# xyfJASON/ctrlora

Hardware: AMD Instinct MI355X
Metric: 512x512 LoRA-finetune images/sec (higher is better)
Workload: dtype bf16; 1 GPU; ctrlora_finetune_sd15_rank128.yaml, canny-style latent hint, 512x512 (latent 64x64), per-GPU batch 8, bf16 storage / fp32 accumulate, synthetic latents + random-init weights, LoRA+zero-conv+norm trainables, fused AdamW; global_batch=8, parallelism=dp1, lora_rank=128, launch=hipGraph replay, gemm_launch_table_entries=215

## Files before the change

ctrlora_amd/csrc/gemm.hip:

```cpp
#include <type_traits>
#include "gemm.h"
#include <algorithm>
#include <cstring>
#include <map>
#include <vector>
#include <utility>
#include "mma.h"
#include "gemm_epi.h"

namespace cl {

static void* g_ws = nullptr;
static long g_ws_bytes = 0;
struct StreamWs { hipStream_t st; void* p; long bytes; };
static StreamWs g_sws[4] = {};
static thread_local hipStream_t t_stream = nullptr;
void gemm_set_workspace(void* p, long bytes) { g_ws = p; g_ws_bytes = bytes; }
int gemm_set_stream_workspace(hipStream_t st, void* p, long bytes) {
  for (auto& e : g_sws) if (e.st == st || e.p == nullptr) { e.st = st; e.p = p; e.bytes = bytes; return CL_OK; }
  return CL_EINVAL;
}
static void ws_for(hipStream_t st, void** p, long* bytes) {
  for (auto& e : g_sws) if (e.p && e.st == st) { *p = e.p; *bytes = e.bytes; return; }
  *p = g_ws; *bytes = g_ws_bytes;
}
void gemm_get_workspace(void** p, long* bytes) { ws_for(t_stream, p, bytes); }
void gemm_get_workspace_for(hipStream_t st, void** p, long* bytes) { ws_for(st, p, bytes); }

int g_gemm_tag_on = 0;
static thread_local int t_tag = 0;
struct TagEntry { long v[12]; };
static std::vector<TagEntry> g_tags;
int gemm_cur_tag() { return t_tag; }
void gemm_tag_note(long real_wgs, int wg_size) {
  if (t_tag > 0 && t_tag <= (int)g_tags.size()) { g_tags[t_tag - 1].v[9] = real_wgs; g_tags[t_tag - 1].v[10] = wg_size; }
}
int gemm_tag_count() { return (int)g_tags.size(); }
void gemm_tag_clear() { g_tags.clear(); t_tag = 0; }
int gemm_tag_get(int i, long* out) {
  if (i < 0 || i >= (int)g_tags.size()) return CL_EINVAL;
  for (int k = 0; k < 12; ++k) out[k] = g_tags[i].v[k];
// ... 72 lines not shown
          }
        }
        __syncthreads();
        continue;
      }
    }
    __builtin_amdgcn_wave_barrier();
    asm volatile("s_waitcnt lgkmcnt(0)" ::: "memory");
#pragma unroll
    for (int it = 0; it < ITERS; ++it) {
      const int rr = it * RPI + lane / LPR;
      const int cg = (lane % LPR) * 8;
      const int grow = row0 + ps * 32 + rr;
      const int gcol = col0 + cg;
      if (lane < RPI * LPR && rr < FPP * 16 && grow < p.M && gcol < p.N) {
        float v[8];
        const float4 s0 = *reinterpret_cast<const float4*>(&stg[rr * EST + cg]);
        const float4 s1 = *reinterpret_cast<const float4*>(&stg[rr * EST + cg + 4]);
        v[0] = s0.x; v[1] = s0.y; v[2] = s0.z; v[3] = s0.w;
        v[4] = s1.x; v[5] = s1.y; v[6] = s1.z; v[7] = s1.w;
        if (slab) {
          store8(slab + ((long)zsplit * p.M + grow) * p.N + gcol, v);
        } else if (p.act != 77) {
          epilogue8<T>(e, v, grow, gcol);
        }
      }
    }
    __builtin_amdgcn_wave_barrier();
  }
}

template <typename T, int BM, int BN, int WGM, int WGN, int KSUB, int R>
__global__ __launch_bounds__(WGM * WGN * 64, 2) void gemm_kernel(GemmParams p, int tiles_m, int tiles_n,
                                                              float* __restrict__ slab) {
  constexpr int NW = WGM * WGN;
  constexpr int KPB = 64 / (int)sizeof(T);
  constexpr int WM = BM / WGM, WN = BN / WGN, FM = WM / 16, FN = WN / 16;
  constexpr int AG = BM / 16, BG = BN / 16;
  constexpr int AJ = AG / NW, BJ = (BG + NW - 1) / NW;
  constexpr int G = AJ + BJ;
  constexpr int D = R - KSUB;
  constexpr int SLOT = (AG + BG) * 1024;
  constexpr int EST = WN + 4;
  constexpr int EROWS = (FM >= 2) ? 32 : 16;
  constexpr int EPI_BYTES = NW * EROWS * EST * 4;
  constexpr int SMEM = (R * SLOT > EPI_BYTES) ? R * SLOT : EPI_BYTES;
  static_assert(AG % NW == 0 && WM % 16 == 0 && WN % 16 == 0 && WN % 8 == 0, "tile shape");
  static_assert(D >= KSUB && D >= 1, "ring too shallow");
  static_assert(FM == 1 || FM % 2 == 0, "FM");
  extern __shared__ __attribute__((aligned(16))) char smem[];

  const int tid = threadIdx.x, lane = tid & 63;
  const int wave = __builtin_amdgcn_readfirstlane(tid >> 6);
  const int wm = wave / WGN, wn = wave % WGN;

  const int nt = tiles_m * tiles_n;
  if ((int)blockIdx.x >= nt * max(p.splitk, 1)) return;
  int pid = blockIdx.x;
  const int zsplit = pid / nt;
  pid -= zsplit * nt;
  {
    const int q = nt >> 3, r = nt & 7, xcd = pid & 7, idx = pid >> 3;
    pid = (xcd < r ? xcd * (q + 1) : r * (q + 1) + (xcd - r) * q) + idx;
  }
  const int m0 = (pid / tiles_n) * BM, n0 = (pid % tiles_n) * BN;

  const int taps = (p.mode == GEMM_LINEAR) ? 1 : 9;
  const int cpt = p.K1 / KPB;
  const int ks1 = taps * cpt;
  const int ks2 = p.K2 / KPB;
  int kbeg = 0, kend = ks1 + ks2;
  if (p.splitk > 1) {
    const int per = (kend + p.splitk - 1) / p.splitk;
    kbeg = zsplit * per;
    kend = min(kend, kbeg + per);
  }

  const int lrow = lane >> 2;
  const int lchk = (lane & 3) * 16;
  const char* a1[AJ]; const char* a2[AJ];
  int ab[AJ], ay[AJ], ax[AJ];
#pragma unroll
  for (int j = 0; j < AJ; ++j) {
    int r = m0 + (j * NW + wave) * 16 + lrow;
    r = min(r, p.M - 1);
    a2[j] = p.A2 ? (const char*)p.A2 + ((long)r * p.lda2 + (p.a2_group_n ? (long)(n0 / p.a2_group_n) * p.K2 : 0)) * sizeof(T) + lchk
                 : nullptr;
    if (p.mode == GEMM_LINEAR) {
      a1[j] = (const char*)p.A1 + ((long)r * p.lda1 + (p.a1_group_n ? (long)(n0 / p.a1_group_n) * p.K1 : 0)) * sizeof(T) + lchk;
      ab[j] = ay[j] = ax[j] = 0;
    } else {
      const int ox = r % p.Wout; const int t = r / p.Wout;
      ax[j] = ox; ay[j] = t % p.Hout; ab[j] = t / p.Hout;
      a1[j] = (const char*)p.A1 + lchk;
    }
  }
  const char* w1[BJ]; const char* w2[BJ];
  int bgrp[BJ];
#pragma unroll
  for (int j = 0; j < BJ; ++j) {
    bgrp[j] = min(j * NW + wave, BG - 1);
    int n = n0 + bgrp[j] * 16 + lrow;
    n = min(n, p.N - 1);
    w1[j] = (const char*)p.W1 + ((long)n * p.ldw1) * sizeof(T) + lchk;
    w2[j] = p.W2 ? (const char*)p.W2 + ((long)n * p.ldw2) * sizeof(T) + lchk : nullptr;
  }
  const char* zpage = (const char*)p.zero_page + lchk;

  auto issue = [&](int kt, int slot) {
    char* As = smem + slot * SLOT;
    char* Bs = As + AG * 1024;
    const bool seg2 = kt >= ks1;
    const long koff = (long)(seg2 ? kt - ks1 : kt) * 64;
    if (seg2 || p.mode == GEMM_LINEAR) {
#pragma unroll
      for (int j = 0; j < AJ; ++j) glds16((seg2 ? a2[j] : a1[j]) + koff, As + (j * NW + wave) * 1024);
    } else {
      const int tap = kt / cpt, cc = kt - tap * cpt;
      const int ky = tap / 3, kx = tap - ky * 3;
      const int sy = (p.mode == GEMM_CONV_S2 || p.mode == GEMM_CONV_S2A) ? 2 : 1;
      const int po = (p.mode == GEMM_CONV_S2A) ? 0 : 1;
      const bool virt = (p.mode == GEMM_CONV_UP2) | (p.mode == GEMM_CONV_T2);
#pragma unroll
      for (int j = 0; j < AJ; ++j) {
        const int vy = ay[j] * sy + ky - po, vx = ax[j] * sy + kx - po;
        bool ok; int iy, ix;
        if (virt) {
          ok = ((unsigned)vy < (unsigned)(2 * p.Hin)) & ((unsigned)vx < (unsigned)(2 * p.Win));
          if (p.mode == GEMM_CONV_T2) ok = ok & !((vy | vx) & 1);
          iy = vy >> 1; ix = vx >> 1;
        } else {
          ok = ((unsigned)vy < (unsigned)p.Hin) & ((unsigned)vx < (unsigned)p.Win);
          iy = vy; ix = vx;
        }
        const long pix = ((long)ab[j] * p.Hin + iy) * p.Win + ix;
        const char* src = ok ? a1[j] + (pix * p.lda1 + (long)cc * KPB) * sizeof(T) : zpage;
        glds16(src, As + (j * NW + wave) * 1024);
      }
    }
#pragma unroll
    for (int j = 0; j < BJ; ++j) glds16((seg2 ? w2[j] : w1[j]) + koff, Bs + bgrp[j] * 1024);
  };

  f32x4_t acc[FM][FN];
#pragma unroll
  for (int i = 0; i < FM; ++i)
#pragma unroll
    for (int j = 0; j < FN; ++j) acc[i][j] = f32x4_t{0.f, 0.f, 0.f, 0.f};

  const int frag_off = ((lane & 15) * 4 + (lane >> 4)) * 16;
  const uint32_t lds_base = (uint32_t)(uintptr_t)smem;
  const uint32_t a_frag = lds_base + (wm * FM) * 1024 + frag_off;
// ... 50 lines not shown
      const bool two = it + 1 < total;
      read_frags(it % R, af0, bf0);
      wait_frags(af0, bf0);
      if (two) read_frags((it + 1) % R, af1, bf1);
      __builtin_amdgcn_sched_barrier(0);
      mma_all(af0, bf0);
      if (two) {
        wait_frags(af1, bf1);
        mma_all(af1, bf1);
      }
    }
  }
  __syncthreads();

  store_tile<T, FM, FN, (WGN == 2 && FN == 5)>(p, acc, reinterpret_cast<float*>(smem) + wave * (EROWS * EST),
                                               m0 + wm * WM, n0 + wn * WN, lane, slab, zsplit, wn,
                                               reinterpret_cast<float*>(smem) + (wave ^ 1) * (EROWS * EST));
}

enum { FL_LINEAR = 0, FL_CONV_S1 = 1, FL_CONV_ANY = 2 };

#ifdef FL_TIMING
__device__ unsigned long long* g_fl_timing = nullptr;
#define FL_STAMP(i) do { if (g_fl_timing && threadIdx.x == 0) { g_fl_timing[(long)vpid * 8 + (i)] = __builtin_amdgcn_s_memtime(); \
    if ((i) == 0) { g_fl_timing[(long)vpid * 8 + 5] = __builtin_amdgcn_s_getreg((31 << 11) | 4);     \
                    g_fl_timing[(long)vpid * 8 + 6] = __builtin_amdgcn_s_getreg((31 << 11) | 20); } } } while (0)
void fl_timing_set(unsigned long long* buf) { (void)hipMemcpyToSymbol(HIP_SYMBOL(g_fl_timing), &buf, sizeof(buf)); }
#else
#define FL_STAMP(i) do { } while (0)
#endif

template <typename T, int BM, int BN, int WGM, int WGN, int MODE, int R, int PRIO>
__device__ __forceinline__ void fl_tile(const GemmParams& p, int tiles_m, int tiles_n, float* __restrict__ slab,
                                        int vpid, char* smem) {
  constexpr int NW = WGM * WGN;
  static_assert(R == 2 || R == 3, "ring depth");
  constexpr int KPS = 128 / (int)sizeof(T);
  constexpr int WM = BM / WGM, WN = BN / WGN, FM = WM / 16, FN = WN / 16;
  constexpr int AI = BM / 8, BI = BN / 8;
  constexpr int AJ = AI / NW, BJ = (BI + NW - 1) / NW;
  constexpr int G = AJ + BJ;
  constexpr int SLOT = (AI + BI) * 1024;
  constexpr int EST = WN + 4;
  constexpr int EROWS = (FM >= 2) ? 32 : 16;
  static_assert(AI % NW == 0 && WM % 16 == 0 && WN % 16 == 0, "tile shape");
  static_assert(NW * EROWS * EST * 4 <= R * SLOT, "epilogue staging must fit in the ring");
  FL_STAMP(0);

  const int tid = threadIdx.x, lane = tid & 63;
  const int wave = __builtin_amdgcn_readfirstlane(tid >> 6);
  const int wm = wave / WGN, wn = wave % WGN;

  const int nt = tiles_m * tiles_n;
  int pid = vpid;
  const int zsplit = pid / nt;
  pid -= zsplit * nt;
  {
    const int q = nt >> 3, r = nt & 7, xcd = pid & 7, idx = pid >> 3;
    pid = (xcd < r ? xcd * (q + 1) : r * (q + 1) + (xcd - r) * q) + idx;
  }
  const int m0 = (pid / tiles_n) * BM, n0 = (pid % tiles_n) * BN;

  const int cpt = p.K1 / KPS;
  int ph_mq = 0, ph = 0, ph_ntx = 3, ph_dy0 = 0, ph_dx0 = 0, ntaps = (MODE == FL_CONV_ANY && p.mode == GEMM_CONV_S2K4) ? 16 : 9;
  long ph_woff = 0;
  if constexpr (MODE == FL_CONV_ANY) {
    if (gemm_phase_mode(p.mode)) {
      ph_mq = p.B * p.Hin * p.Win;
      ph = m0 / ph_mq;
      const int a = ph >> 1, b = ph & 1;
      if (p.mode == GEMM_CONV_UP2P) { ph_ntx = 2; ntaps = 4; ph_dy0 = a - 1; ph_dx0 = b - 1; ph_woff = (long)ph * 4 * p.N * p.K1; }
      else { ph_ntx = 1 + b; ntaps = (1 + a) * (1 + b); ph_woff = (long)p.N * p.K1 * (ph == 0 ? 0 : ph == 1 ? 1 : ph == 2 ? 3 : 5); }
    }
  }
  const long ldw1 = ph_mq ? (long)ntaps * p.K1 : p.ldw1;
  const int ks1 = (MODE == FL_LINEAR ? 1 : ntaps) * cpt;
  const int ks2 = (MODE == FL_LINEAR) ? p.K2 / KPS : 0;
  int kbeg = 0, kend = ks1 + ks2;
  if (p.splitk > 1) {
    const int per = (kend + p.splitk - 1) / p.splitk;
    kbeg = zsplit * per;
    kend = min(kend, kbeg + per);
  }
  const int total = kend - kbeg;

  const int lrow = lane >> 3, lslot = lane & 7;
  const char* pa[AJ];
  const char* a2[AJ];
  uint32_t vmask[AJ];
  int ab[AJ], ay[AJ], ax[AJ];
#pragma unroll
  for (int j = 0; j < AJ; ++j) {
    const int inst = j * NW + wave;
    const int chunk = (lslot ^ (((inst & 1) << 2) | (lrow >> 1))) * 16;
    int r = m0 + inst * 8 + lrow;
    r = min(r, p.M - 1);
    a2[j] = nullptr; vmask[j] = 0; ab[j] = ay[j] = ax[j] = 0;
    if constexpr (MODE == FL_LINEAR) {
      const bool in2 = kbeg >= ks1;
      a2[j] = p.A2 ? (const char*)p.A2 + ((long)r * p.lda2 + (p.a2_group_n ? (long)(n0 / p.a2_group_n) * p.K2 : 0)) * sizeof(T) + chunk
                   : nullptr;
      pa[j] = in2 ? a2[j] + (long)(kbeg - ks1) * 128
                  : (const char*)p.A1 + ((long)r * p.lda1 + (p.a1_group_n ? (long)(n0 / p.a1_group_n) * p.K1 : 0)) * sizeof(T) +
                        chunk + (long)kbeg * 128;
    } else {
      const int rq = ph_mq ? r - ph * ph_mq : r;
      const int gw = ph_mq ? p.Win : p.Wout, gh = ph_mq ? p.Hin : p.Hout;
      const int ox = rq % gw; const int t = rq / gw;
      const int oy = t % gh, ob = t / gh;
      if constexpr (MODE == FL_CONV_S1) {
        pa[j] = (const char*)p.A1 + ((((long)ob * p.Hin + oy) * p.Win + ox) * p.lda1) * sizeof(T) + chunk;
        uint32_t m = 0;
#pragma unroll
        for (int tp = 0; tp < 9; ++tp) {
          const int vy = oy + tp / 3 - 1, vx = ox + tp % 3 - 1;
          if (((unsigned)vy < (unsigned)p.Hin) & ((unsigned)vx < (unsigned)p.Win)) m |= 1u << tp;
        }
        vmask[j] = m;
      } else {
        pa[j] = (const char*)p.A1 + chunk;
        ax[j] = ox; ay[j] = oy; ab[j] = ob;
      }
    }
  }
  const char* pw[BJ]; const char* w2[BJ];
  int binst[BJ];
#pragma unroll
  for (int j = 0; j < BJ; ++j) {
    binst[j] = min(j * NW + wave, BI - 1);
    const int chunk = (lslot ^ (((binst[j] & 1) << 2) | (lrow >> 1))) * 16;
    int n = n0 + binst[j] * 8 + lrow;
    n = min(n, p.N - 1);
    w2[j] = (MODE == FL_LINEAR && p.W2) ? (const char*)p.W2 + ((long)n * p.ldw2) * sizeof(T) + chunk : nullptr;
    pw[j] = (MODE == FL_LINEAR && kbeg >= ks1)
                ? w2[j] + (long)(kbeg - ks1) * 128
                : (const char*)p.W1 + (ph_woff + (long)n * ldw1) * sizeof(T) + chunk + (long)kbeg * 128;
  }
  const char* zpage = (const char*)p.zero_page + lslot * 16;

  int kt_next = kbeg;
  int tap = (MODE == FL_LINEAR) ? 0 : kbeg / cpt;
  int cc = (MODE == FL_LINEAR) ? 0 : kbeg - tap * cpt;
  const long pixb = (long)p.lda1 * sizeof(T);
  long tapoff = 0;
  const char* cur[AJ];
#pragma unroll
  for (int j = 0; j < AJ; ++j) cur[j] = nullptr;
  if constexpr (MODE == FL_CONV_S1) {
    tapoff = ((long)(tap / 3 - 1) * p.Win + (tap % 3 - 1)) * pixb;
#pragma unroll
    for (int j = 0; j < AJ; ++j)
      cur[j] = ((vmask[j] >> tap) & 1u) ? pa[j] + tapoff + (long)cc * 128 : zpage + (long)cc * 128;
  }

  auto issue_a = [&](int slot) {
    char* As = smem + slot * SLOT;
    if constexpr (MODE == FL_LINEAR) {
      if (ks2 && kt_next == ks1) {
#pragma unroll
        for (int j = 0; j < AJ; ++j) pa[j] = a2[j];
      }
#pragma unroll
      for (int j = 0; j < AJ; ++j) { glds16(pa[j], As + (j * NW + wave) * 1024); pa[j] += 128; }
    } else if constexpr (MODE == FL_CONV_S1) {
      if (cc == 0) {
#pragma unroll
        for (int j = 0; j < AJ; ++j) cur[j] = ((vmask[j] >> tap) & 1u) ? pa[j] + tapoff : zpage;
      }
#pragma unroll
      for (int j = 0; j < AJ; ++j) { glds16(cur[j], As + (j * NW + wave) * 1024); cur[j] += 128; }
    } else {
      const bool k4 = p.mode == GEMM_CONV_S2K4;
      const int ky = k4 ? tap >> 2 : tap / 3, kx = k4 ? tap & 3 : tap - ky * 3;
      const int sy = (p.mode == GEMM_CONV_S2 || p.mode == GEMM_CONV_S2A || k4) ? 2 : 1;
      const int po = (p.mode == GEMM_CONV_S2A) ? 0 : 1;
      const bool virt = (p.mode == GEMM_CONV_UP2) | (p.mode == GEMM_CONV_T2);
      const int pty = ph_ntx == 2 ? tap >> 1 : tap, ptx = ph_ntx == 2 ? tap & 1 : 0;
#pragma unroll
      for (int j = 0; j < AJ; ++j) {
        const int vy = ph_mq ? ay[j] + ph_dy0 + pty : ay[j] * sy + ky - po;
        const int vx = ph_mq ? ax[j] + ph_dx0 + ptx : ax[j] * sy + kx - po;
        bool ok; int iy, ix;
        if (virt) {
          ok = ((unsigned)vy < (unsigned)(2 * p.Hin)) & ((unsigned)vx < (unsigned)(2 * p.Win));
          if (p.mode == GEMM_CONV_T2) ok = ok & !((vy | vx) & 1);
          iy = vy >> 1; ix = vx >> 1;
        } else {
          ok = ((unsigned)vy < (unsigned)p.Hin) & ((unsigned)vx < (unsigned)p.Win);
          iy = vy; ix = vx;
        }
        const long pix = ((long)ab[j] * p.Hin + iy) * p.Win + ix;
        const char* src = ok ? pa[j] + pix * pixb + (long)cc * 128 : zpage;
        glds16(src, As + (j * NW + wave) * 1024);
      }
    }
  };
  auto issue_b = [&](int slot) {
    char* Bs = smem + slot * SLOT + AI * 1024;
    if constexpr (MODE == FL_LINEAR) {
      if (ks2 && kt_next == ks1) {
#pragma unroll
        for (int j = 0; j < BJ; ++j) pw[j] = w2[j];
      }
    } else if constexpr (MODE == FL_CONV_S1) {
      const bool wrap = cc + 1 == cpt;
      cc = wrap ? 0 : cc + 1;
      tap += wrap ? 1 : 0;
      const int ky = (tap * 11) >> 5;
      tapoff = ((long)(ky - 1) * p.Win + (tap - 3 * ky - 1)) * pixb;
    } else {
      if (++cc == cpt) { cc = 0; ++tap; }
    }
#pragma unroll
    for (int j = 0; j < BJ; ++j) { glds16(pw[j], Bs + binst[j] * 1024); pw[j] += 128; }
    ++kt_next;
  };
  auto issue_next = [&](int slot) { issue_a(slot); issue_b(slot); };
  FL_STAMP(1);

  f32x4_t acc[FM][FN];
#pragma unroll
  for (int i = 0; i < FM; ++i)
#pragma unroll
    for (int j = 0; j < FN; ++j) acc[i][j] = f32x4_t{0.f, 0.f, 0.f, 0.f};

  const int lr = lane & 15, g = lane >> 4;
  const uint32_t lds_base = (uint32_t)(uintptr_t)smem;
  const uint32_t frag0 = lr * 128 + ((g ^ (lr >> 1)) * 16);
  const uint32_t a_base = lds_base + (wm * FM) * 2048;
  const uint32_t b_base = lds_base + AI * 1024 + (wn * FN) * 2048;

  auto read_frags = [&](int slot, int half, u32x4_t (&af)[FM], u32x4_t (&bfr)[FN]) {
    const uint32_t off = (half ? (frag0 ^ 64u) : frag0) + slot * SLOT;
    const uint32_t aa = a_base + off, ba = b_base + off;
#pragma unroll
    for (int i = 0; i < FM; ++i)
      asm volatile("ds_read_b128 %0, %1 offset:%2" : "=v"(af[i]) : "v"(aa), "i"(i * 2048) : "memory");
#pragma unroll
    for (int j = 0; j < FN; ++j)
      asm volatile("ds_read_b128 %0, %1 offset:%2" : "=v"(bfr[j]) : "v"(ba), "i"(j * 2048) : "memory");
  };
  auto wait_frags = [&](u32x4_t (&af)[FM], u32x4_t (&bfr)[FN]) {
    asm volatile("s_waitcnt lgkmcnt(0)" ::: "memory");
#pragma unroll
    for (int i = 0; i < FM; ++i) asm volatile("" : "+v"(af[i]));
#pragma unroll
    for (int j = 0; j < FN; ++j) asm volatile("" : "+v"(bfr[j]));
    __builtin_amdgcn_sched_barrier(0);
  };
  auto mma_all = [&](const u32x4_t (&af)[FM], const u32x4_t (&bfr)[FN]) {
#pragma unroll
    for (int i = 0; i < FM; ++i)
#pragma unroll
      for (int j = 0; j < FN; ++j) Mma<T>::run(af[i], bfr[j], acc[i][j]);
  };

  u32x4_t fa[FM], fb[FN], ga[FM], gb[FN];
  int slot = 0;
  if constexpr (PRIO == 4) {
    static_assert(PRIO != 4 || R == 3, "ping-pong needs the 3-slot ring");
    const int grp = wave / (NW / 2);
    issue_next(0);
    if (total > 1) { issue_next(1); wait_vm<G>(); } else { wait_vm<0>(); }
    __builtin_amdgcn_s_barrier();
    if (grp == 1) __builtin_amdgcn_s_barrier();
    __builtin_amdgcn_sched_barrier(0);
    auto stage4 = [&](auto ISSUE) {
      constexpr bool issue = decltype(ISSUE)::value;
      const int slot1 = (slot == R - 1) ? 0 : slot + 1;
      const int slot2 = (slot1 == R - 1) ? 0 : slot1 + 1;
      read_frags(slot, 0, fa, fb);
      read_frags(slot, 1, ga, gb);
      if constexpr (issue) issue_next(slot2);
      __builtin_amdgcn_sched_barrier(0);
      asm volatile("s_waitcnt lgkmcnt(0)" ::: "memory");
      if constexpr (issue) wait_vm<G>(); else wait_vm<0>();
      __builtin_amdgcn_s_barrier();
      __builtin_amdgcn_sched_barrier(0);
#pragma unroll
      for (int i = 0; i < FM; ++i) { asm volatile("" : "+v"(fa[i])); asm volatile("" : "+v"(ga[i])); }
#pragma unroll
      for (int j = 0; j < FN; ++j) { asm volatile("" : "+v"(fb[j])); asm volatile("" : "+v"(gb[j])); }
      __builtin_amdgcn_s_setprio(1);
      mma_all(fa, fb);
      mma_all(ga, gb);
      __builtin_amdgcn_s_setprio(0);
      __builtin_amdgcn_sched_barrier(0);
      __builtin_amdgcn_s_barrier();
      __builtin_amdgcn_sched_barrier(0);
      slot = slot1;
    };
    int s = 0;
    for (; s + 2 < total; ++s) stage4(std::true_type{});
    for (; s < total; ++s) stage4(std::false_type{});
    if (grp == 0) __builtin_amdgcn_s_barrier();
  } else if constexpr (PRIO == 3) {
    static_assert(PRIO != 3 || R == 3, "ping-pong needs the 3-slot ring");
    const int grp = wave / (NW / 2);
    issue_next(0);
    if (total > 1) issue_next(1);
    if (total > 2) { issue_a(2); wait_vm<G + AJ>(); } else if (total > 1) { wait_vm<G>(); } else { wait_vm<0>(); }
    __builtin_amdgcn_s_barrier();
    FL_STAMP(2);
    __builtin_amdgcn_sched_barrier(0);
    read_frags(0, 0, fa, fb);
    wait_frags(fa, fb);
    if (grp == 1) __builtin_amdgcn_s_barrier();
    __builtin_amdgcn_sched_barrier(0);
    auto stage3 = [&](auto IB_, auto IA_, bool has_next) {
      constexpr bool IB = decltype(IB_)::value, IA = decltype(IA_)::value;
      const int slot1 = (slot == R - 1) ? 0 : slot + 1;
      const int slot2 = (slot1 == R - 1) ? 0 : slot1 + 1;
#ifndef FLP_NOLDS
      read_frags(slot, 1, ga, gb);
#endif
      if constexpr (IB) issue_b(slot2);
      __builtin_amdgcn_sched_barrier(0);
      asm volatile("s_waitcnt lgkmcnt(0)" ::: "memory");
      if constexpr (IB) wait_vm<G>(); else wait_vm<0>();
      __builtin_amdgcn_s_barrier();
      __builtin_amdgcn_sched_barrier(0);
      __builtin_amdgcn_s_setprio(1);
      mma_all(fa, fb);
      __builtin_amdgcn_s_setprio(0);
      __builtin_amdgcn_sched_barrier(0);
      __builtin_amdgcn_s_barrier();
      __builtin_amdgcn_sched_barrier(0);
#ifndef FLP_NOLDS
      if (has_next) read_frags(slot1, 0, fa, fb);
#endif
      if constexpr (IA) issue_a(slot);
      __builtin_amdgcn_sched_barrier(0);
      asm volatile("s_waitcnt lgkmcnt(0)" ::: "memory");
      __builtin_amdgcn_s_barrier();
      __builtin_amdgcn_sched_barrier(0);
#pragma unroll
      for (int i = 0; i < FM; ++i) asm volatile("" : "+v"(ga[i]));
#pragma unroll
      for (int j = 0; j < FN; ++j) asm volatile("" : "+v"(gb[j]));
      __builtin_amdgcn_s_setprio(1);
      mma_all(ga, gb);
      __builtin_amdgcn_s_setprio(0);
      __builtin_amdgcn_sched_barrier(0);
      __builtin_amdgcn_s_barrier();
      __builtin_amdgcn_sched_barrier(0);
#pragma unroll
      for (int i = 0; i < FM; ++i) asm volatile("" : "+v"(fa[i]));
#pragma unroll
      for (int j = 0; j < FN; ++j) asm volatile("" : "+v"(fb[j]));
      slot = slot1;
    };
    int s = 0;
#ifdef FLP_NODMA
    for (; s + 3 < total; ++s) stage3(std::false_type{}, std::false_type{}, true);
#endif
    for (; s + 3 < total; ++s) stage3(std::true_type{}, std::true_type{}, true);
    for (; s + 2 < total; ++s) stage3(std::true_type{}, std::false_type{}, true);
    for (; s < total; ++s) stage3(std::false_type{}, std::false_type{}, s + 1 < total);
    if (grp == 0) __builtin_amdgcn_s_barrier();
  } else if constexpr (PRIO == 2) {
    static_assert(PRIO != 2 || R == 3, "split issue needs the 3-slot ring");
    issue_next(0);
    if (total > 1) { issue_next(1); wait_vm<G>(); } else { wait_vm<0>(); }
    __builtin_amdgcn_s_barrier();
    __builtin_amdgcn_sched_barrier(0);
    read_frags(0, 0, fa, fb);
    wait_frags(fa, fb);
    auto stage2 = [&](auto ISSUE, bool has_next) {
      constexpr bool issue = decltype(ISSUE)::value;
      const int slot1 = (slot == R - 1) ? 0 : slot + 1;
      const int slot2 = (slot1 == R - 1) ? 0 : slot1 + 1;
      read_frags(slot, 1, ga, gb);
      __builtin_amdgcn_sched_barrier(0);
      mma_all(fa, fb);
      if constexpr (issue) issue_a(slot2);
      __builtin_amdgcn_sched_barrier(0);
      asm volatile("s_waitcnt lgkmcnt(0)" ::: "memory");
      if constexpr (issue) wait_vm<AJ>(); else wait_vm<0>();
      __builtin_amdgcn_s_barrier();
      __builtin_amdgcn_sched_barrier(0);
      if (has_next) read_frags(slot1, 0, fa, fb);
      __builtin_amdgcn_sched_barrier(0);
#pragma unroll
      for (int i = 0; i < FM; ++i) asm volatile("" : "+v"(ga[i]));
#pragma unroll
      for (int j = 0; j < FN; ++j) asm volatile("" : "+v"(gb[j]));
      mma_all(ga, gb);
      if constexpr (issue) issue_b(slot2);
      wait_frags(fa, fb);
      slot = slot1;
    };
    int s = 0;
    for (; s + 2 < total; ++s) stage2(std::true_type{}, true);
    for (; s < total; ++s) stage2(std::false_type{}, s + 1 < total);
  } else {
  issue_next(0);
  if (total > 1) {
    issue_next(1);
    wait_vm<G>();
  } else {
    wait_vm<0>();
  }
  __builtin_amdgcn_s_barrier();
  FL_STAMP(2);
  __builtin_amdgcn_sched_barrier(0);
  read_frags(0, 0, fa, fb);
  wait_frags(fa, fb);

  auto stage = [&](auto ISSUE, bool has_next) {
    constexpr bool issue = decltype(ISSUE)::value;
    const int slot1 = (slot == R - 1) ? 0 : slot + 1;
    const int slot2 = (slot1 == R - 1) ? 0 : slot1 + 1;
    read_frags(slot, 1, ga, gb);
    __builtin_amdgcn_sched_barrier(0);
    mma_all(fa, fb);
    if constexpr (issue && R == 3) issue_next(slot2);
    __builtin_amdgcn_sched_barrier(0);
    asm volatile("s_waitcnt lgkmcnt(0)" ::: "memory");
    if constexpr (issue && R == 3) wait_vm<G>(); else wait_vm<0>();
    __builtin_amdgcn_s_barrier();
    __builtin_amdgcn_sched_barrier(0);
    if (has_next) read_frags(slot1, 0, fa, fb);
    __builtin_amdgcn_sched_barrier(0);
#pragma unroll
    for (int i = 0; i < FM; ++i) asm volatile("" : "+v"(ga[i]));
#pragma unroll
    for (int j = 0; j < FN; ++j) asm volatile("" : "+v"(gb[j]));
    if constexpr (PRIO == 1) __builtin_amdgcn_s_setprio(1);
    mma_all(ga, gb);
    if constexpr (PRIO == 1) __builtin_amdgcn_s_setprio(0);
    if constexpr (issue && R == 2) issue_next(slot);
    wait_frags(fa, fb);
    slot = slot1;
  };
  int s = 0;
  for (; s + 2 < total; ++s) stage(std::true_type{}, true);
  for (; s < total; ++s) stage(std::false_type{}, s + 1 < total);
  }
  FL_STAMP(3);
  __syncthreads();

  store_tile<T, FM, FN, (WGN == 2 && FN == 5)>(p, acc, reinterpret_cast<float*>(smem) + wave * (EROWS * EST),
                                               m0 + wm * WM, n0 + wn * WN, lane, slab, zsplit, wn,
                                               reinterpret_cast<float*>(smem) + (wave ^ 1) * (EROWS * EST));
  FL_STAMP(4);
#ifdef FL_TIMING
  if (g_fl_timing) { asm volatile("s_waitcnt vmcnt(0)" ::: "memory"); FL_STAMP(7); }
#endif
}

template <typename T, int BM, int BN, int WGM, int WGN, int MODE, int R, int PRIO = 0>
__global__ __launch_bounds__(WGM * WGN * 64, 2) void gemm_fl_kernel(GemmParams p, int tiles_m, int tiles_n,
                                                                 float* __restrict__ slab) {
  extern __shared__ __attribute__((aligned(16))) char smem[];
  if ((int)blockIdx.x >= tiles_m * tiles_n * max(p.splitk, 1)) return;
  fl_tile<T, BM, BN, WGM, WGN, MODE, R, PRIO>(p, tiles_m, tiles_n, slab, (int)blockIdx.x, smem);
}

template <typename T, int BM, int BN, int WGM, int WGN, int MODE, int R, int PRIO = 0>
__global__ __launch_bounds__(WGM * WGN * 64, 2) void gemm_fl_persist_kernel(GemmParams p, int tiles_m, int tiles_n,
                                                                         float* __restrict__ slab, int nvirt,
                                                                         int stagger) {
  extern __shared__ __attribute__((aligned(16))) char smem[];
  if (stagger > 0 && blockIdx.x >= gridDim.x / 2) {
    const unsigned long long t0 = __builtin_amdgcn_s_memtime();
    while (__builtin_amdgcn_s_memtime() - t0 < (unsigned long long)stagger) __builtin_amdgcn_s_sleep(8);
  }
  for (int v = blockIdx.x; v < nvirt; v += gridDim.x) {
    fl_tile<T, BM, BN, WGM, WGN, MODE, R, PRIO>(p, tiles_m, tiles_n, slab, v, smem);
    __syncthreads();
  }
}

template <typename T>
__global__ __launch_bounds__(256) void splitk_reduce_kernel(GemmParams p, const float* __restrict__ slab, int splits) {
  const EpiArgs e = epi_of(p);
  if (p.act == ACT_GEGLU) {
    const int o8 = p.N / 16;
    const long total = (long)p.M * o8;
    for (long i = (long)blockIdx.x * blockDim.x + threadIdx.x; i < total; i += (long)gridDim.x * blockDim.x) {
      const int grow = (int)(i / o8), ocol = (int)(i % o8) * 8;
      const int vcol = (ocol / 80) * 160 + ocol % 80;
      float v[8] = {0.f, 0.f, 0.f, 0.f, 0.f, 0.f, 0.f, 0.f}, g[8] = {0.f, 0.f, 0.f, 0.f, 0.f, 0.f, 0.f, 0.f};
      for (int z = 0; z < splits; ++z) {
        float t[8];
        load8(slab + ((long)z * p.M + grow) * p.N + vcol, t);
#pragma unroll
        for (int k = 0; k < 8; ++k) v[k] += t[k];
        load8(slab + ((long)z * p.M + grow) * p.N + vcol + 80, t);
#pragma unroll
        for (int k = 0; k < 8; ++k) g[k] += t[k];
      }
      if (e.bias) {
#pragma unroll
        for (int k = 0; k < 8; ++k) { v[k] += e.bias[vcol + k]; g[k] += e.bias[vcol + 80 + k]; }
      }
#pragma unroll
      for (int k = 0; k < 8; ++k) v[k] *= gelu_f(g[k]);
      if (p.out_f32) store8(reinterpret_cast<float*>(e.C) + (long)grow * e.ldc + ocol, v);
      else store8(reinterpret_cast<T*>(e.C) + (long)grow * e.ldc + ocol, v);
    }
    return;
// ... 35 lines not shown
  const int kpb = 64 / (int)sizeof(T);
  const int tm = (p.M + BM - 1) / BM, tn = (p.N + BN - 1) / BN;
  const long tiles = (long)tm * tn;
  const int ksub = ((p.mode == GEMM_LINEAR ? 1 : 9) * p.K1 + p.K2) / kpb;
  float* slab = nullptr;
  if (p.atomic) {
    if (p.splitk < 1) p.splitk = 1;
    if (p.splitk > ksub) p.splitk = ksub > 0 ? ksub : 1;
  } else {
    int sk = 1;
    void* wsp; long wsb;
    ws_for(stream, &wsp, &wsb);
    if (t_force_sk > 0) {
      sk = wsp ? t_force_sk : 1;
      if (sk > ksub) sk = ksub > 0 ? ksub : 1;
      while (sk > 1 && (long)sk * p.M * p.N * 4 > wsb) --sk;
    } else if (p.splitk <= 1 && tiles < 160 && ksub >= 32 && wsp) {
      sk = (int)((256 + tiles - 1) / tiles);
      const int minsub = p.M <= 64 ? g_tiny_m_minsub : 16;
      if (sk > ksub / minsub) sk = ksub / minsub;
      if (sk > 16) sk = 16;
      while (sk > 1 && (long)sk * p.M * p.N * 4 > wsb) --sk;
      if (sk < 1) sk = 1;
    }
    p.splitk = sk;
    if (sk > 1) slab = reinterpret_cast<float*>(wsp);
  }
  if (p.splitk > 1) {
    const int per = (ksub + p.splitk - 1) / p.splitk;
    p.splitk = (ksub + per - 1) / per;
  }
  const long grid = tiles * p.splitk;
  gemm_tag_note(grid, NW * 64);
  hipLaunchKernelGGL(kern, dim3((unsigned)(grid + t_tag)), dim3(NW * 64), SMEM, stream, p, tm, tn, slab);
  if (slab) {
    const long total = (long)p.M * (p.N / 8);
    int rg = (int)((total + 255) / 256); if (rg > 4096) rg = 4096;
    hipLaunchKernelGGL((splitk_reduce_kernel<T>), dim3(rg), dim3(256), 0, stream, p, slab, p.splitk);
  }
  CL_CHECK_LAUNCH();
  return CL_OK;
}

static int pick_splitk(GemmParams& p, long tiles, int steps, int want, int min_steps, float** slab,
                       hipStream_t stream) {
  void* wsp; long wsb;
  ws_for(stream, &wsp, &wsb);
  *slab = nullptr;
  if (p.atomic) {
    if (p.splitk < 1) p.splitk = 1;
    if (p.splitk > steps) p.splitk = steps > 0 ? steps : 1;
  } else {
    int sk = 1;
    if (t_force_sk > 0) {
      sk = wsp ? t_force_sk : 1;
      if (sk > steps) sk = steps > 0 ? steps : 1;
      while (sk > 1 && (long)sk * p.M * p.N * 4 > wsb) --sk;
    } else if (tiles < want && steps >= 2 * min_steps && wsp) {
      sk = (int)((want + tiles - 1) / tiles);
      if (sk > steps / min_steps) sk = steps / min_steps;
      if (sk > 32) sk = 32;
      while (sk > 1 && (long)sk * p.M * p.N * 4 > wsb) --sk;
      if (sk < 1) sk = 1;
    }
    p.splitk = sk;
    if (sk > 1) *slab = reinterpret_cast<float*>(wsp);
  }
// ... 17 lines not shown
  static int n = 0;
  if (!n) {
    int dev = 0; hipDeviceProp_t pr;
    if (hipGetDevice(&dev) != hipSuccess || hipGetDeviceProperties(&pr, dev) != hipSuccess) return 256;
    n = pr.multiProcessorCount > 0 ? pr.multiProcessorCount : 256;
  }
  return n;
}

template <typename T, int BM, int BN, int WGM, int WGN, int MODE, int R, int PRIO = 0, bool PERSIST = false>
static int launch_fl_mode(const GemmParams& p0, hipStream_t stream) {
  constexpr int NW = WGM * WGN;
  constexpr int SMEM = R * (BM / 8 + BN / 8) * 1024;
  static bool attr_set = false;
  if (!attr_set) {
    const void* k;
    if constexpr (PERSIST) k = reinterpret_cast<const void*>(&gemm_fl_persist_kernel<T, BM, BN, WGM, WGN, MODE, R, PRIO>);
    else k = reinterpret_cast<const void*>(&gemm_fl_kernel<T, BM, BN, WGM, WGN, MODE, R, PRIO>);
    if (SMEM > 65536 && hipFuncSetAttribute(k, hipFuncAttributeMaxDynamicSharedMemorySize, SMEM) != hipSuccess)
      return CL_ELAUNCH;
    attr_set = true;
  }
  if ((p0.a1_group_n && p0.a1_group_n % BN) || (p0.a2_group_n && p0.a2_group_n % BN)) return CL_EINVAL;
  GemmParams p = p0;
  const int kps = 128 / (int)sizeof(T);
  const int tm = (p.M + BM - 1) / BM, tn = (p.N + BN - 1) / BN;
  const long tiles = (long)tm * tn;
  const int steps = ((MODE == FL_LINEAR ? 1 : p.mode == GEMM_CONV_UP2P ? 4 : p.mode == GEMM_CONV_S2K4 ? 16 : 9) * p.K1 + p.K2) / kps;
  float* slab;
  if (gemm_phase_mode(p.mode) && (p.B * p.Hin * p.Win) % BM) return CL_EINVAL;
  if (p.mode == GEMM_CONV_T2P) { p.splitk = 1; slab = nullptr; }
  else pick_splitk(p, tiles, steps, R == 3 ? (BM == 128 ? g_fl128_split_want : 256) : 512, 4, &slab, stream);
  const long nvirt = tiles * p.splitk;
  if constexpr (PERSIST) {
    long grid = (long)device_cus() * (SMEM > 80 * 1024 ? 1 : 2);
    grid -= grid % 8;
    if (grid > nvirt) grid = nvirt;
    if (grid < nvirt) grid -= grid % 8;
    if (grid < 1) grid = nvirt;
    gemm_tag_note(grid, NW * 64);
    hipLaunchKernelGGL((gemm_fl_persist_kernel<T, BM, BN, WGM, WGN, MODE, R, PRIO>), dim3((unsigned)(grid + t_tag)), dim3(NW * 64),
                       SMEM, stream, p, tm, tn, slab, (int)nvirt, (SMEM <= 80 * 1024 && grid == 2L * device_cus() && nvirt >= 2 * grid) ? g_fl_persist_stagger : 0);
  } else {
    gemm_tag_note(nvirt, NW * 64);
    hipLaunchKernelGGL((gemm_fl_kernel<T, BM, BN, WGM, WGN, MODE, R, PRIO>), dim3((unsigned)(nvirt + t_tag)), dim3(NW * 64), SMEM,
                       stream, p, tm, tn, slab);
  }
  if (slab) {
    const long total = (long)p.M * (p.N / 8);
    int rg = (int)((total + 255) / 256); if (rg > 4096) rg = 4096;
    hipLaunchKernelGGL((splitk_reduce_kernel<T>), dim3(rg), dim3(256), 0, stream, p, slab, p.splitk);
  }
  CL_CHECK_LAUNCH();
  return CL_OK;
}

template <typename T, int BM, int BN, int WGM, int WGN, int R, int PRIO = 0, bool PERSIST = false>
static int launch_fl(const GemmParams& p, hipStream_t stream) {
  if (p.mode == GEMM_LINEAR) return launch_fl_mode<T, BM, BN, WGM, WGN, FL_LINEAR, R, PRIO, PERSIST>(p, stream);
  if constexpr (PERSIST) return CL_EINVAL;
  if (p.K2) return CL_EINVAL;
  if (p.mode == GEMM_CONV_S1) return launch_fl_mode<T, BM, BN, WGM, WGN, FL_CONV_S1, R, PRIO>(p, stream);
  return launch_fl_mode<T, BM, BN, WGM, WGN, FL_CONV_ANY, R>(p, stream);
}

int g_gemm_force_cfg = -1;
int g_gemm_xs_rules = 1;
int g_fl128_split_want = 128;
int g_tiny_m_minsub = 8;

int g_fl_persist_stagger = 0;
int g_gemm_force_splitk = 0;

struct TuneKey {
  int v[7];
  bool operator<(const TuneKey& o) const { return std::lexicographical_compare(v, v + 7, o.v, o.v + 7); }
};
static std::map<TuneKey, std::pair<int, int>> g_tune;

// ... 231 lines not shown
```

Before: 238.5 images/s.

## Precompute magic-number divisors and issue weight tile loads before A-address setup

Replaces runtime integer divisions and modulos in the GEMM tile prologue and conv im2col address math with host-precomputed multiply-shift fast division (TileDiv passed as a kernel argument). It also hoists the first two B (weight) DMA loads ahead of the A-operand address computation so weight fetches are in flight during prologue math, and changes the prologue waits to count only A loads. This targets prologue latency on small, many-tile GEMMs. It adds kernel-argument size and relies on the fast-division range assumptions plus the correctness of the reordered wait counts.

Result: no change. 239.2 images/s, median of 6 (+0.3%).

```diff
diff --git a/ctrlora_amd/csrc/fastdiv.h b/ctrlora_amd/csrc/fastdiv.h
--- /dev/null
+++ b/ctrlora_amd/csrc/fastdiv.h
@@ -0,0 +1,55 @@
+#pragma once
+#include <cstdint>
+
+#if defined(__HIPCC__)
+#define CL_FD_HD __host__ __device__ __forceinline__
+#else
+#define CL_FD_HD inline
+#endif
+
+namespace cl {
+
+constexpr uint32_t kFastDivMaxDividend = 0x7fffffffu;
+
+struct FastDiv { uint32_t mul, shift; };
+
+inline FastDiv fastdiv_make(uint32_t d) {
+  if (d == 0) d = 1;
+  uint32_t s = 0;
+  while (s < 32 && (uint64_t(1) << s) < d) ++s;
+  const uint64_t m = ((uint64_t(1) << 32) * ((uint64_t(1) << s) - d)) / d + 1;
+  return FastDiv{(uint32_t)m, s};
+}
+
+CL_FD_HD uint32_t fastdiv_mulhi(uint32_t a, uint32_t b) {
+#if defined(__HIP_DEVICE_COMPILE__)
+  return __umulhi(a, b);
+#else
+  return (uint32_t)(((uint64_t)a * b) >> 32);
+#endif
+}
+
+CL_FD_HD uint32_t fastdiv_q(uint32_t n, FastDiv f) { return (fastdiv_mulhi(n, f.mul) + n) >> f.shift; }
+CL_FD_HD int fastdiv_q(int n, FastDiv f) { return (int)fastdiv_q((uint32_t)n, f); }
+
+struct TileDiv {
+  FastDiv nt;
+  FastDiv tiles_n;
+  FastDiv gw, gh;
+  FastDiv ph_mq;
+  FastDiv cpt;
+  FastDiv a1g, a2g;
+  FastDiv splitk;
+};
+
+inline TileDiv tilediv_make(long nt, int tiles_n, int gw, int gh, long ph_mq, int cpt, int a1g, int a2g, int splitk) {
+  TileDiv d;
+  d.nt = fastdiv_make((uint32_t)nt); d.tiles_n = fastdiv_make((uint32_t)tiles_n);
+  d.gw = fastdiv_make((uint32_t)gw); d.gh = fastdiv_make((uint32_t)gh);
+  d.ph_mq = fastdiv_make((uint32_t)ph_mq); d.cpt = fastdiv_make((uint32_t)cpt);
+  d.a1g = fastdiv_make((uint32_t)a1g); d.a2g = fastdiv_make((uint32_t)a2g);
+  d.splitk = fastdiv_make((uint32_t)(splitk > 1 ? splitk : 1));
+  return d;
+}
+
+}
diff --git a/ctrlora_amd/csrc/gemm.hip b/ctrlora_amd/csrc/gemm.hip
--- a/ctrlora_amd/csrc/gemm.hip
+++ b/ctrlora_amd/csrc/gemm.hip
@@ -7,6 +7,7 @@
 #include <utility>
 #include "mma.h"
 #include "gemm_epi.h"
+#include "fastdiv.h"
 
 namespace cl {
 
@@ -145,7 +146,7 @@
 
 template <typename T, int BM, int BN, int WGM, int WGN, int KSUB, int R>
 __global__ __launch_bounds__(WGM * WGN * 64, 2) void gemm_kernel(GemmParams p, int tiles_m, int tiles_n,
-                                                              float* __restrict__ slab) {
+                                                              float* __restrict__ slab, TileDiv dv) {
   constexpr int NW = WGM * WGN;
   constexpr int KPB = 64 / (int)sizeof(T);
   constexpr int WM = BM / WGM, WN = BN / WGN, FM = WM / 16, FN = WN / 16;
@@ -170,21 +171,22 @@
   const int nt = tiles_m * tiles_n;
   if ((int)blockIdx.x >= nt * max(p.splitk, 1)) return;
   int pid = blockIdx.x;
-  const int zsplit = pid / nt;
+  const int zsplit = fastdiv_q(pid, dv.nt);
   pid -= zsplit * nt;
   {
     const int q = nt >> 3, r = nt & 7, xcd = pid & 7, idx = pid >> 3;
     pid = (xcd < r ? xcd * (q + 1) : r * (q + 1) + (xcd - r) * q) + idx;
   }
-  const int m0 = (pid / tiles_n) * BM, n0 = (pid % tiles_n) * BN;
+  const int tile_m = fastdiv_q(pid, dv.tiles_n);
+  const int m0 = tile_m * BM, n0 = (pid - tile_m * tiles_n) * BN;
 
   const int taps = (p.mode == GEMM_LINEAR) ? 1 : 9;
-  const int cpt = p.K1 / KPB;
+  const int cpt = (int)((unsigned)p.K1 / KPB);
   const int ks1 = taps * cpt;
-  const int ks2 = p.K2 / KPB;
+  const int ks2 = (int)((unsigned)p.K2 / KPB);
   int kbeg = 0, kend = ks1 + ks2;
   if (p.splitk > 1) {
-    const int per = (kend + p.splitk - 1) / p.splitk;
+    const int per = fastdiv_q(kend + p.splitk - 1, dv.splitk);
     kbeg = zsplit * per;
     kend = min(kend, kbeg + per);
   }
@@ -193,18 +195,20 @@
   const int lchk = (lane & 3) * 16;
   const char* a1[AJ]; const char* a2[AJ];
   int ab[AJ], ay[AJ], ax[AJ];
+  const long g1off = p.a1_group_n ? (long)fastdiv_q(n0, dv.a1g) * p.K1 : 0;
+  const long g2off = p.a2_group_n ? (long)fastdiv_q(n0, dv.a2g) * p.K2 : 0;
 #pragma unroll
   for (int j = 0; j < AJ; ++j) {
     int r = m0 + (j * NW + wave) * 16 + lrow;
     r = min(r, p.M - 1);
-    a2[j] = p.A2 ? (const char*)p.A2 + ((long)r * p.lda2 + (p.a2_group_n ? (long)(n0 / p.a2_group_n) * p.K2 : 0)) * sizeof(T) + lchk
+    a2[j] = p.A2 ? (const char*)p.A2 + ((long)r * p.lda2 + g2off) * sizeof(T) + lchk
                  : nullptr;
     if (p.mode == GEMM_LINEAR) {
-      a1[j] = (const char*)p.A1 + ((long)r * p.lda1 + (p.a1_group_n ? (long)(n0 / p.a1_group_n) * p.K1 : 0)) * sizeof(T) + lchk;
+      a1[j] = (const char*)p.A1 + ((long)r * p.lda1 + g1off) * sizeof(T) + lchk;
       ab[j] = ay[j] = ax[j] = 0;
     } else {
-      const int ox = r % p.Wout; const int t = r / p.Wout;
-      ax[j] = ox; ay[j] = t % p.Hout; ab[j] = t / p.Hout;
+      const int t = fastdiv_q(r, dv.gw);
+      ax[j] = r - t * p.Wout; ab[j] = fastdiv_q(t, dv.gh); ay[j] = t - ab[j] * p.Hout;
       a1[j] = (const char*)p.A1 + lchk;
     }
   }
@@ -229,8 +233,8 @@
 #pragma unroll
       for (int j = 0; j < AJ; ++j) glds16((seg2 ? a2[j] : a1[j]) + koff, As + (j * NW + wave) * 1024);
     } else {
-      const int tap = kt / cpt, cc = kt - tap * cpt;
-      const int ky = tap / 3, kx = tap - ky * 3;
+      const int tap = fastdiv_q(kt, dv.cpt), cc = kt - tap * cpt;
+      const int ky = (tap * 11) >> 5, kx = tap - ky * 3;
       const int sy = (p.mode == GEMM_CONV_S2 || p.mode == GEMM_CONV_S2A) ? 2 : 1;
       const int po = (p.mode == GEMM_CONV_S2A) ? 0 : 1;
       const bool virt = (p.mode == GEMM_CONV_UP2) | (p.mode == GEMM_CONV_T2);
@@ -347,7 +351,7 @@
 
 template <typename T, int BM, int BN, int WGM, int WGN, int MODE, int R, int PRIO>
 __device__ __forceinline__ void fl_tile(const GemmParams& p, int tiles_m, int tiles_n, float* __restrict__ slab,
-                                        int vpid, char* smem) {
+                                        int vpid, char* smem, const TileDiv& dv) {
   constexpr int NW = WGM * WGN;
   static_assert(R == 2 || R == 3, "ring depth");
   constexpr int KPS = 128 / (int)sizeof(T);
@@ -368,21 +372,22 @@
 
   const int nt = tiles_m * tiles_n;
   int pid = vpid;
-  const int zsplit = pid / nt;
+  const int zsplit = fastdiv_q(pid, dv.nt);
   pid -= zsplit * nt;
   {
     const int q = nt >> 3, r = nt & 7, xcd = pid & 7, idx = pid >> 3;
     pid = (xcd < r ? xcd * (q + 1) : r * (q + 1) + (xcd - r) * q) + idx;
   }
-  const int m0 = (pid / tiles_n) * BM, n0 = (pid % tiles_n) * BN;
-
-  const int cpt = p.K1 / KPS;
+  const int tile_m = fastdiv_q(pid, dv.tiles_n);
+  const int m0 = tile_m * BM, n0 = (pid - tile_m * tiles_n) * BN;
+
+  const int cpt = (int)((unsigned)p.K1 / KPS);
   int ph_mq = 0, ph = 0, ph_ntx = 3, ph_dy0 = 0, ph_dx0 = 0, ntaps = (MODE == FL_CONV_ANY && p.mode == GEMM_CONV_S2K4) ? 16 : 9;
   long ph_woff = 0;
   if constexpr (MODE == FL_CONV_ANY) {
     if (gemm_phase_mode(p.mode)) {
       ph_mq = p.B * p.Hin * p.Win;
-      ph = m0 / ph_mq;
+      ph = fastdiv_q(m0, dv.ph_mq);
       const int a = ph >> 1, b = ph & 1;
       if (p.mode == GEMM_CONV_UP2P) { ph_ntx = 2; ntaps = 4; ph_dy0 = a - 1; ph_dx0 = b - 1; ph_woff = (long)ph * 4 * p.N * p.K1; }
       else { ph_ntx = 1 + b; ntaps = (1 + a) * (1 + b); ph_woff = (long)p.N * p.K1 * (ph == 0 ? 0 : ph == 1 ? 1 : ph == 2 ? 3 : 5); }
@@ -390,20 +395,55 @@
   }
   const long ldw1 = ph_mq ? (long)ntaps * p.K1 : p.ldw1;
   const int ks1 = (MODE == FL_LINEAR ? 1 : ntaps) * cpt;
-  const int ks2 = (MODE == FL_LINEAR) ? p.K2 / KPS : 0;
+  const int ks2 = (MODE == FL_LINEAR) ? (int)((unsigned)p.K2 / KPS) : 0;
   int kbeg = 0, kend = ks1 + ks2;
   if (p.splitk > 1) {
-    const int per = (kend + p.splitk - 1) / p.splitk;
+    const int per = fastdiv_q(kend + p.splitk - 1, dv.splitk);
     kbeg = zsplit * per;
     kend = min(kend, kbeg + per);
   }
   const int total = kend - kbeg;
 
   const int lrow = lane >> 3, lslot = lane & 7;
+  const char* pw[BJ]; const char* w2[BJ];
+  int binst[BJ];
+#pragma unroll
+  for (int j = 0; j < BJ; ++j) {
+    binst[j] = min(j * NW + wave, BI - 1);
+    const int chunk = (lslot ^ (((binst[j] & 1) << 2) | (lrow >> 1))) * 16;
+    int n = n0 + binst[j] * 8 + lrow;
+    n = min(n, p.N - 1);
+    w2[j] = (MODE == FL_LINEAR && p.W2) ? (const char*)p.W2 + ((long)n * p.ldw2) * sizeof(T) + chunk : nullptr;
+    pw[j] = (MODE == FL_LINEAR && kbeg >= ks1)
+                ? w2[j] + (long)(kbeg - ks1) * 128
+                : (const char*)p.W1 + (ph_woff + (long)n * ldw1) * sizeof(T) + chunk + (long)kbeg * 128;
+  }
+  auto dma_b = [&](int slot) {
+    char* Bs = smem + slot * SLOT + AI * 1024;
+#pragma unroll
+    for (int j = 0; j < BJ; ++j) { glds16(pw[j], Bs + binst[j] * 1024); pw[j] += 128; }
+  };
+  dma_b(0);
+  if (total > 1) {
+    if constexpr (MODE == FL_LINEAR) {
+      if (ks2 && kbeg + 1 == ks1) {
+#pragma unroll
+        for (int j = 0; j < BJ; ++j) pw[j] = w2[j];
+      }
+    }
+    dma_b(1);
+  }
+  __builtin_amdgcn_sched_barrier(0);
+
   const char* pa[AJ];
   const char* a2[AJ];
   uint32_t vmask[AJ];
   int ab[AJ], ay[AJ], ax[AJ];
+  long g1off = 0, g2off = 0;
+  if constexpr (MODE == FL_LINEAR) {
+    if (p.a1_group_n) g1off = (long)fastdiv_q(n0, dv.a1g) * p.K1;
+    if (p.a2_group_n) g2off = (long)fastdiv_q(n0, dv.a2g) * p.K2;
+  }
 #pragma unroll
   for (int j = 0; j < AJ; ++j) {
     const int inst = j * NW + wave;
@@ -413,16 +453,18 @@
     a2[j] = nullptr; vmask[j] = 0; ab[j] = ay[j] = ax[j] = 0;
     if constexpr (MODE == FL_LINEAR) {
       const bool in2 = kbeg >= ks1;
-      a2[j] = p.A2 ? (const char*)p.A2 + ((long)r * p.lda2 + (p.a2_group_n ? (long)(n0 / p.a2_group_n) * p.K2 : 0)) * sizeof(T) + chunk
+      a2[j] = p.A2 ? (const char*)p.A2 + ((long)r * p.lda2 + g2off) * sizeof(T) + chunk
                    : nullptr;
       pa[j] = in2 ? a2[j] + (long)(kbeg - ks1) * 128
-                  : (const char*)p.A1 + ((long)r * p.lda1 + (p.a1_group_n ? (long)(n0 / p.a1_group_n) * p.K1 : 0)) * sizeof(T) +
+                  : (const char*)p.A1 + ((long)r * p.lda1 + g1off) * sizeof(T) +
                         chunk + (long)kbeg * 128;
     } else {
       const int rq = ph_mq ? r - ph * ph_mq : r;
       const int gw = ph_mq ? p.Win : p.Wout, gh = ph_mq ? p.Hin : p.Hout;
-      const int ox = rq % gw; const int t = rq / gw;
-      const int oy = t % gh, ob = t / gh;
+      const int t = fastdiv_q(rq, dv.gw);
+      const int ox = rq - t * gw;
+      const int ob = fastdiv_q(t, dv.gh);
+      const int oy = t - ob * gh;
       if constexpr (MODE == FL_CONV_S1) {
         pa[j] = (const char*)p.A1 + ((((long)ob * p.Hin + oy) * p.Win + ox) * p.lda1) * sizeof(T) + chunk;
         uint32_t m = 0;
@@ -438,23 +480,10 @@
       }
     }
   }
-  const char* pw[BJ]; const char* w2[BJ];
-  int binst[BJ];
-#pragma unroll
-  for (int j = 0; j < BJ; ++j) {
-    binst[j] = min(j * NW + wave, BI - 1);
-    const int chunk = (lslot ^ (((binst[j] & 1) << 2) | (lrow >> 1))) * 16;
-    int n = n0 + binst[j] * 8 + lrow;
-    n = min(n, p.N - 1);
-    w2[j] = (MODE == FL_LINEAR && p.W2) ? (const char*)p.W2 + ((long)n * p.ldw2) * sizeof(T) + chunk : nullptr;
-    pw[j] = (MODE == FL_LINEAR && kbeg >= ks1)
-                ? w2[j] + (long)(kbeg - ks1) * 128
-                : (const char*)p.W1 + (ph_woff + (long)n * ldw1) * sizeof(T) + chunk + (long)kbeg * 128;
-  }
   const char* zpage = (const char*)p.zero_page + lslot * 16;
 
   int kt_next = kbeg;
-  int tap = (MODE == FL_LINEAR) ? 0 : kbeg / cpt;
+  int tap = (MODE == FL_LINEAR) ? 0 : fastdiv_q(kbeg, dv.cpt);
   int cc = (MODE == FL_LINEAR) ? 0 : kbeg - tap * cpt;
   const long pixb = (long)p.lda1 * sizeof(T);
   long tapoff = 0;
@@ -462,7 +491,8 @@
 #pragma unroll
   for (int j = 0; j < AJ; ++j) cur[j] = nullptr;
   if constexpr (MODE == FL_CONV_S1) {
-    tapoff = ((long)(tap / 3 - 1) * p.Win + (tap % 3 - 1)) * pixb;
+    const int ky0 = (tap * 11) >> 5;
+    tapoff = ((long)(ky0 - 1) * p.Win + (tap - 3 * ky0 - 1)) * pixb;
 #pragma unroll
     for (int j = 0; j < AJ; ++j)
       cur[j] = ((vmask[j] >> tap) & 1u) ? pa[j] + tapoff + (long)cc * 128 : zpage + (long)cc * 128;
@@ -486,7 +516,7 @@
       for (int j = 0; j < AJ; ++j) { glds16(cur[j], As + (j * NW + wave) * 1024); cur[j] += 128; }
     } else {
       const bool k4 = p.mode == GEMM_CONV_S2K4;
-      const int ky = k4 ? tap >> 2 : tap / 3, kx = k4 ? tap & 3 : tap - ky * 3;
+      const int ky = k4 ? tap >> 2 : (tap * 11) >> 5, kx = k4 ? tap & 3 : tap - ky * 3;
       const int sy = (p.mode == GEMM_CONV_S2 || p.mode == GEMM_CONV_S2A || k4) ? 2 : 1;
       const int po = (p.mode == GEMM_CONV_S2A) ? 0 : 1;
       const bool virt = (p.mode == GEMM_CONV_UP2) | (p.mode == GEMM_CONV_T2);
@@ -510,27 +540,30 @@
       }
     }
   };
-  auto issue_b = [&](int slot) {
-    char* Bs = smem + slot * SLOT + AI * 1024;
-    if constexpr (MODE == FL_LINEAR) {
-      if (ks2 && kt_next == ks1) {
-#pragma unroll
-        for (int j = 0; j < BJ; ++j) pw[j] = w2[j];
-      }
-    } else if constexpr (MODE == FL_CONV_S1) {
+  auto advance = [&]() {
+    if constexpr (MODE == FL_CONV_S1) {
       const bool wrap = cc + 1 == cpt;
       cc = wrap ? 0 : cc + 1;
       tap += wrap ? 1 : 0;
       const int ky = (tap * 11) >> 5;
       tapoff = ((long)(ky - 1) * p.Win + (tap - 3 * ky - 1)) * pixb;
-    } else {
+    } else if constexpr (MODE == FL_CONV_ANY) {
       if (++cc == cpt) { cc = 0; ++tap; }
     }
-#pragma unroll
-    for (int j = 0; j < BJ; ++j) { glds16(pw[j], Bs + binst[j] * 1024); pw[j] += 128; }
+  };
+  auto issue_b = [&](int slot) {
+    if constexpr (MODE == FL_LINEAR) {
+      if (ks2 && kt_next == ks1) {
+#pragma unroll
+        for (int j = 0; j < BJ; ++j) pw[j] = w2[j];
+      }
+    }
+    advance();
+    dma_b(slot);
     ++kt_next;
   };
   auto issue_next = [&](int slot) { issue_a(slot); issue_b(slot); };
+  auto fill_a = [&](int slot) { issue_a(slot); advance(); ++kt_next; };
   FL_STAMP(1);
 
   f32x4_t acc[FM][FN];
@@ -575,8 +608,8 @@
   if constexpr (PRIO == 4) {
     static_assert(PRIO != 4 || R == 3, "ping-pong needs the 3-slot ring");
     const int grp = wave / (NW / 2);
-    issue_next(0);
-    if (total > 1) { issue_next(1); wait_vm<G>(); } else { wait_vm<0>(); }
+    fill_a(0);
+    if (total > 1) { fill_a(1); wait_vm<AJ>(); } else { wait_vm<0>(); }
     __builtin_amdgcn_s_barrier();
     if (grp == 1) __builtin_amdgcn_s_barrier();
     __builtin_amdgcn_sched_barrier(0);
@@ -612,9 +645,9 @@
   } else if constexpr (PRIO == 3) {
     static_assert(PRIO != 3 || R == 3, "ping-pong needs the 3-slot ring");
     const int grp = wave / (NW / 2);
-    issue_next(0);
-    if (total > 1) issue_next(1);
-    if (total > 2) { issue_a(2); wait_vm<G + AJ>(); } else if (total > 1) { wait_vm<G>(); } else { wait_vm<0>(); }
+    fill_a(0);
+    if (total > 1) fill_a(1);
+    if (total > 2) { issue_a(2); wait_vm<2 * AJ>(); } else if (total > 1) { wait_vm<AJ>(); } else { wait_vm<0>(); }
     __builtin_amdgcn_s_barrier();
     FL_STAMP(2);
     __builtin_amdgcn_sched_barrier(0);
@@ -675,8 +708,8 @@
     if (grp == 0) __builtin_amdgcn_s_barrier();
   } else if constexpr (PRIO == 2) {
     static_assert(PRIO != 2 || R == 3, "split issue needs the 3-slot ring");
-    issue_next(0);
-    if (total > 1) { issue_next(1); wait_vm<G>(); } else { wait_vm<0>(); }
+    fill_a(0);
+    if (total > 1) { fill_a(1); wait_vm<AJ>(); } else { wait_vm<0>(); }
     __builtin_amdgcn_s_barrier();
     __builtin_amdgcn_sched_barrier(0);
     read_frags(0, 0, fa, fb);
@@ -709,10 +742,10 @@
     for (; s + 2 < total; ++s) stage2(std::true_type{}, true);
     for (; s < total; ++s) stage2(std::false_type{}, s + 1 < total);
   } else {
-  issue_next(0);
+  fill_a(0);
   if (total > 1) {
-    issue_next(1);
-    wait_vm<G>();
+    fill_a(1);
+    wait_vm<AJ>();
   } else {
     wait_vm<0>();
   }
@@ -766,23 +799,23 @@
 
 template <typename T, int BM, int BN, int WGM, int WGN, int MODE, int R, int PRIO = 0>
 __global__ __launch_bounds__(WGM * WGN * 64, 2) void gemm_fl_kernel(GemmParams p, int tiles_m, int tiles_n,
-                                                                 float* __restrict__ slab) {
+                                                                 float* __restrict__ slab, TileDiv dv) {
   extern __shared__ __attribute__((aligned(16))) char smem[];
   if ((int)blockIdx.x >= tiles_m * tiles_n * max(p.splitk, 1)) return;
-  fl_tile<T, BM, BN, WGM, WGN, MODE, R, PRIO>(p, tiles_m, tiles_n, slab, (int)blockIdx.x, smem);
+  fl_tile<T, BM, BN, WGM, WGN, MODE, R, PRIO>(p, tiles_m, tiles_n, slab, (int)blockIdx.x, smem, dv);
 }
 
 template <typename T, int BM, int BN, int WGM, int WGN, int MODE, int R, int PRIO = 0>
 __global__ __launch_bounds__(WGM * WGN * 64, 2) void gemm_fl_persist_kernel(GemmParams p, int tiles_m, int tiles_n,
                                                                          float* __restrict__ slab, int nvirt,
-                                                                         int stagger) {
+                                                                         int stagger, TileDiv dv) {
   extern __shared__ __attribute__((aligned(16))) char smem[];
   if (stagger > 0 && blockIdx.x >= gridDim.x / 2) {
     const unsigned long long t0 = __builtin_amdgcn_s_memtime();
     while (__builtin_amdgcn_s_memtime() - t0 < (unsigned long long)stagger) __builtin_amdgcn_s_sleep(8);
   }
   for (int v = blockIdx.x; v < nvirt; v += gridDim.x) {
-    fl_tile<T, BM, BN, WGM, WGN, MODE, R, PRIO>(p, tiles_m, tiles_n, slab, v, smem);
+    fl_tile<T, BM, BN, WGM, WGN, MODE, R, PRIO>(p, tiles_m, tiles_n, slab, v, smem, dv);
     __syncthreads();
   }
 }
@@ -884,7 +917,8 @@
   }
   const long grid = tiles * p.splitk;
   gemm_tag_note(grid, NW * 64);
-  hipLaunchKernelGGL(kern, dim3((unsigned)(grid + t_tag)), dim3(NW * 64), SMEM, stream, p, tm, tn, slab);
+  const TileDiv dv = tilediv_make(tiles, tn, p.Wout, p.Hout, 0, p.K1 / kpb, p.a1_group_n, p.a2_group_n, p.splitk);
+  hipLaunchKernelGGL(kern, dim3((unsigned)(grid + t_tag)), dim3(NW * 64), SMEM, stream, p, tm, tn, slab, dv);
   if (slab) {
     const long total = (long)p.M * (p.N / 8);
     int rg = (int)((total + 255) / 256); if (rg > 4096) rg = 4096;
@@ -968,6 +1002,9 @@
   if (p.mode == GEMM_CONV_T2P) { p.splitk = 1; slab = nullptr; }
   else pick_splitk(p, tiles, steps, R == 3 ? (BM == 128 ? g_fl128_split_want : 256) : 512, 4, &slab, stream);
   const long nvirt = tiles * p.splitk;
+  const bool phm = gemm_phase_mode(p.mode);
+  const TileDiv dv = tilediv_make(tiles, tn, phm ? p.Win : p.Wout, phm ? p.Hin : p.Hout, phm ? (long)p.B * p.Hin * p.Win : 0, p.K1 / kps,
+                                  p.a1_group_n, p.a2_group_n, p.splitk);
   if constexpr (PERSIST) {
     long grid = (long)device_cus() * (SMEM > 80 * 1024 ? 1 : 2);
     grid -= grid % 8;
@@ -976,11 +1013,11 @@
     if (grid < 1) grid = nvirt;
     gemm_tag_note(grid, NW * 64);
     hipLaunchKernelGGL((gemm_fl_persist_kernel<T, BM, BN, WGM, WGN, MODE, R, PRIO>), dim3((unsigned)(grid + t_tag)), dim3(NW * 64),
-                       SMEM, stream, p, tm, tn, slab, (int)nvirt, (SMEM <= 80 * 1024 && grid == 2L * device_cus() && nvirt >= 2 * grid) ? g_fl_persist_stagger : 0);
+                       SMEM, stream, p, tm, tn, slab, (int)nvirt, (SMEM <= 80 * 1024 && grid == 2L * device_cus() && nvirt >= 2 * grid) ? g_fl_persist_stagger : 0, dv);
   } else {
     gemm_tag_note(nvirt, NW * 64);
     hipLaunchKernelGGL((gemm_fl_kernel<T, BM, BN, WGM, WGN, MODE, R, PRIO>), dim3((unsigned)(nvirt + t_tag)), dim3(NW * 64), SMEM,
-                       stream, p, tm, tn, slab);
+                       stream, p, tm, tn, slab, dv);
   }
   if (slab) {
     const long total = (long)p.M * (p.N / 8);
```
